# y2w-oc/CMR-Agent

Measured on AMD Instinct MI355X. Metric: registration iters/sec (KITTI 352x1216 img + 16384 pts, 1 geo forward + 10 agent steps), higher is better.
Workload: dtype f32; 1 GPU; BASELINE.json configs[1]: KittiConfig, batch 8 per GPU, 16384 pts, 352x1216 image, 10 agent steps, fp32, hash-filled weights; batch_per_gpu=8, parallelism=batch sharding, no data-path collective

## Files before the change

cmr_agent_amd/ops.py:

```python
import math
import os

import torch

from . import _lib

ACT_NONE, ACT_RELU, ACT_LRELU, ACT_GELU, ACT_ELU1 = 0, 1, 2, 3, 4
f32 = torch.float32
GRID_Y_MAX = 65535


def _stream():
    return torch.cuda.current_stream().cuda_stream


def _p(t):
    return None if t is None else t.data_ptr()


def _rows(t, name="tensor"):
    if t.dim() != 2 or t.stride(1) != 1 or t.dtype != f32 or not t.is_cuda:
        raise ValueError("%s must be a 2-D float32 device tensor with unit inner stride, got %s %s %s" % (
            name, tuple(t.shape), t.stride(), t.dtype))
    return t
# ... 3 lines not shown
    return t.stride(0) if t.shape[0] > 1 else max(t.stride(0), t.shape[1])


def _i32(t):
    if t is not None and (t.dtype != torch.int32 or not t.is_contiguous()):
        raise ValueError("row-id tensors must be contiguous int32")
    return t


LINEAR_BF16 = os.environ.get("CMR_LINEAR_BF16", "1") != "0"
LINEAR_BF16_MIN_ROWS = 16384
BN_LINEAR_BF16_FWD = os.environ.get("CMR_BN_LINEAR_BF16_FWD", "0") != "0"
BN_LINEAR_BF16_BWD = os.environ.get("CMR_BN_LINEAR_BF16_BWD", "0") != "0"


class fp32_linears:

    def __enter__(self):
        global LINEAR_BF16
        self.old, LINEAR_BF16 = LINEAR_BF16, False

    def __exit__(self, *a):
        global LINEAR_BF16
        LINEAR_BF16 = self.old


_AB_SKIP_LINEAR = os.environ.get("CMR_AB_SKIP_LINEAR", "0") == "1"
_AB_ZERO = {}
if _AB_SKIP_LINEAR:
    import sys as _sys
    print("cmr_agent_amd.ops: CMR_AB_SKIP_LINEAR=1 -- row GEMMs are NOT computed (timing experiment); every result of this process is invalid",
          file=_sys.stderr)


def linear(x1, w, bias=None, x2=None, idx2=None, div2=1, res=None, res_mod=0, act=ACT_NONE, act_param=0.0, out=None):
    _rows(x1, "x1")
    rows, k1 = x1.shape
    n_out, kw = w.shape
    k2 = 0
    if x2 is not None:
        _rows(x2, "x2")
        k2 = x2.shape[1]
    if kw != k1 + k2 or w.stride(1) != 1 or w.stride(0) < kw:
        raise ValueError("weight shape %s / strides %s do not match k1+k2=%d" % (tuple(w.shape), w.stride(), k1 + k2))
    ldw = w.stride(0) if n_out > 1 else kw
    if out is None:
        out = torch.empty((rows, n_out), dtype=f32, device=x1.device)
    _rows(out, "out")
    if res is not None:
        _rows(res, "res")
    if _AB_SKIP_LINEAR:
        key = (rows, n_out, x1.device)
        if key not in _AB_ZERO:
            _AB_ZERO[key] = torch.zeros((rows, n_out), dtype=f32, device=x1.device)
        return _AB_ZERO[key]
    if CONV_BF16 and LINEAR_BF16 and x2 is None and ldw == kw and rows >= LINEAR_BF16_MIN_ROWS and k1 in (32, 64, 128) and n_out <= 128 and n_out % 4 == 0:
        rc = _lib.call("cmr_linear_rows_bf16_f32", _p(x1), _ld(x1), k1, _p(w), kw, _p(bias), _p(res), _ld(res) if res is not None else 0,
                       int(res_mod), _p(out), _ld(out), rows, n_out, act, float(act_param), _stream(), allow_unsupported=True)
        if rc != _lib.UNSUPPORTED:
            return out
    _lib.call("cmr_linear_f32", _p(x1), _ld(x1), k1, _p(x2), _ld(x2) if x2 is not None else 0, k2, _p(_i32(idx2)),
              int(div2), _p(w), ldw, _p(bias), _p(res), _ld(res) if res is not None else 0, int(res_mod), _p(out),
              _ld(out), rows, n_out, act, float(act_param), _stream())
    return out


def cbr_block(x1, w1, b1, w2, b2, wsc, slope, x2=None, idx2=None, div2=1, rows_per_batch=None, want_y=True,
              want_colmax=False):
    _rows(x1, "x1")
    rows, k1 = x1.shape
    kx = k1 + (x2.shape[1] if x2 is not None else 0)
    ch, co = w1.shape[0], w2.shape[0]
    if w1.shape[1] != kx or w2.shape[1] != ch or (wsc is not None and tuple(wsc.shape) != (co, kx)):
        raise ValueError("cbr_block: inconsistent weight shapes")
    rpb = rows if rows_per_batch is None else rows_per_batch
    B = rows // rpb
    if want_colmax and (rpb % 32 or rows % rpb):
        return None
    y = torch.empty((rows, co), dtype=f32, device=x1.device) if want_y else None
    ntiles = (rows + 31) // 32
    part = torch.empty((ntiles, co), dtype=f32, device=x1.device) if want_colmax else None
    s1 = b1.stride(0) if b1.dim() == 2 else 0
    s2 = b2.stride(0) if b2.dim() == 2 else 0
    rc = _lib.call("cmr_cbr_block_bf16_f32" if CONV_BF16 else "cmr_cbr_block_f32", _p(x1), _ld(x1), k1, _p(x2), _ld(x2) if x2 is not None else 0, _p(_i32(idx2)),
                   int(div2), kx, ch, co, _p(w1), _p(b1), s1, _p(w2), _p(b2), s2, _p(wsc), _p(y), co, _p(part), rows, rpb,
                   float(slope), _stream(), allow_unsupported=True)
    if rc == _lib.UNSUPPORTED:
        return None
    cm = None
    if want_colmax == "partials":
        return y, part
    if want_colmax:
        cm = colmax_partials(part, B, rpb // 32)
    return y, cm


def colmax_partials(part, B, tiles_per_batch):
    co = part.shape[1]
    cm = torch.empty((B, co), dtype=f32, device=part.device)
    _lib.call("cmr_colmax_partials_f32", _p(part), _p(cm), B, int(tiles_per_batch), co, _stream())
    return cm


COLMAX_BIAS2 = os.environ.get("CMR_COLMAX_BIAS2", "fp32")


def colmax_bias2(part, B, tiles_per_batch, w1, b1, w2, b2, want_g=False):
    C = part.shape[1]
    n1, n2 = w1.shape[0], w2.shape[0]
    if COLMAX_BIAS2 == "0" or (COLMAX_BIAS2 == "fp32" and CONV_BF16) or C != 64 or n1 % 4 or n2 % 4 or not (w1.is_contiguous() and w2.is_contiguous()) or w1.shape[1] != C or w2.shape[1] != C:
        return None
    y1 = torch.empty((B, n1), dtype=f32, device=part.device)
    y2 = torch.empty((B, n2), dtype=f32, device=part.device)
    g = torch.empty((B, C), dtype=f32, device=part.device) if want_g else None
    rc = _lib.call("cmr_colmax_bias2_f32", _p(part), B, int(tiles_per_batch), C, _p(w1), _p(b1), n1, _p(w2), _p(b2), n2, _p(g), _p(y1), _p(y2), _stream(),
                   allow_unsupported=True)
    return None if rc == _lib.UNSUPPORTED else (y1, y2, g)


def layernorm64(x, gamma, beta, eps, res=None, out=None):
    _rows(x, "x")
    if out is None:
        out = torch.empty((x.shape[0], 64), dtype=f32, device=x.device)
    _lib.call("cmr_layernorm64_f32", _p(x), _ld(x), _p(gamma), _p(beta), float(eps), _p(res),
              _ld(res) if res is not None else 0, _p(out), _ld(out), x.shape[0], _stream())
    return out


CONV_BF16 = False
BF16_CHAINS = True
BF16_STORE = True
STRIDE2_FRAGS = True
WINOGRAD = True
WINO_MIN_TILES = 64


TOWER_CU_BUDGET = 160
TOWER_CU_BUDGET_F32 = 0


TOWER_SLICES_F32 = int(os.environ.get("CMR_TOWER_SLICES", "1"))


import threading

_policy = threading.local()


def _cu_budget():
    return getattr(_policy, "cu_budget", 0)


def _slices():
    return getattr(_policy, "slices", 1)


class conv_slices:

    def __init__(self, n):
        self.n = max(1, int(n))

    def __enter__(self):
        self.old, _policy.slices = _slices(), self.n

    def __exit__(self, *a):
        _policy.slices = self.old


class conv_cu_budget:

    def __init__(self, cus):
        self.cus = max(0, int(cus))

    def __enter__(self):
        self.old, _policy.cu_budget = _cu_budget(), self.cus

    def __exit__(self, *a):
        _policy.cu_budget = self.old


def conv3x3_wino(x, u, bias, cout, slope=1.0, res=None, post=None, pool=1):
    B, H, W, cin = x.shape
    if pool == 2 and (res is not None or post is not None):
        raise ValueError("conv3x3: pool=2 cannot be combined with res / post")
    if not x.is_contiguous() or tuple(u.shape) != (16, cout, cin):
        raise ValueError("conv3x3_wino: bad operand layout")
    hp, wp = (H // 2, W // 2) if pool == 2 else (H, W)
    y = torch.empty((B, hp, wp, cout), dtype=f32, device=x.device)
    _lib.call("cmr_conv3x3_wino_nhwc_f32", _p(x), B, H, W, cin, _p(u), _p(bias), _p(res), _p(post), _p(y), cout,
              float(slope), pool, _cu_budget(), _slices(), _stream())
    return y


def conv3x3_wino_stats(x, u, bias, cout):
    B, H, W, cin = x.shape
    if not (WINOGRAD and u is not None and x.dtype == f32 and x.is_contiguous() and tuple(u.shape) == (16, cout, cin)):
        return None
    parts = int(_lib.load().cmr_conv3x3_wino_stats_parts(B, H, W, cin, cout, _cu_budget(), _slices()))
    if parts <= 0:
        return None
    y = torch.empty((B, H, W, cout), dtype=f32, device=x.device)
    part = torch.empty((parts, 2, cout), dtype=f32, device=x.device)
    _lib.call("cmr_conv3x3_wino_stats_nhwc_f32", _p(x), B, H, W, cin, _p(u), _p(bias), _p(y), cout, _cu_budget(), _slices(), _p(part), parts, _stream())
    return y, part


def conv3x3_wino_bnbwd(dy, u, cout, bn_x, stat, slope):
    B, H, W, cin = dy.shape
    if not (WINOGRAD and u is not None and dy.is_contiguous() and bn_x.is_contiguous() and tuple(u.shape) == (16, cout, cin)
            and tuple(bn_x.shape) == (B, H, W, cout) and tuple(stat.shape) == (4, cout) and 0.0 <= slope <= 1.0):
        return None
# ... 1688 lines not shown
```

cmr_agent_amd/utils/workmodel.py:

```python
import torch

from .. import _lib

FP32_MFMA_PEAK = 157.3e12
HBM_PEAK = 8.0e12
RIDGE = FP32_MFMA_PEAK / HBM_PEAK
F = 4


def _linear(a):
    rows, k1, n = a["rows"], a["k1"], a["n_out"]
    k2 = a["k2"] if a["x2"] else 0
    src2 = 0
    if a["x2"]:
        src2 = rows * k2 if a["idx2"] else max(rows // max(a["div2"], 1), 1) * k2
    by = F * (rows * k1 + src2 + rows * n + n * (k1 + k2) + (rows * n if a["res"] and not a["res_mod"] else 0))
    return 2.0 * rows * (k1 + k2) * n, by


def _cbr(a):
    rows, kx, ch, co, k1 = a["rows"], a["kx"], a["ch"], a["co"], a["k1"]
    w = kx * ch + ch * co + (kx * co if a["wsc"] else 0)
    src2 = 0
    if a["x2"]:
        src2 = rows * (kx - k1) if a["idx2"] else max(rows // max(a["div2"], 1), 1) * (kx - k1)
    return 2.0 * rows * w, F * (rows * k1 + src2 + (rows * co if a["y"] else 0) + w)


def _conv(a, stride=None):
    s = a.get("stride", 1) if stride is None else stride
    B, H, W, ci, co, pool = a["B"], a["H"], a["W"], a["Cin"], a["Cout"], a.get("pool", 1)
    opix = B * ((H - 1) // s + 1) * ((W - 1) // s + 1)
    by = F * (B * H * W * ci + opix * co / (pool * pool) + (opix * co if a["res"] else 0) + 9 * ci * co)
    return 2.0 * 9 * ci * co * opix, by


def _conv_io(a):
    s = a.get("stride", 1)
    B, H, W, ci, co, pool = a["B"], a["H"], a["W"], a["Cin"], a["Cout"], a.get("pool", 1)
    opix = B * ((H - 1) // s + 1) * ((W - 1) // s + 1)
    by = ((2 if a["x_bf16"] else F) * B * H * W * ci + (2 if a["y_bf16"] else F) * opix * co / (pool * pool)
          + (2 if a.get("res_bf16") else F) * (opix * co if a["res"] else 0) + F * 9 * ci * co)
    return 2.0 * 9 * ci * co * opix, by


def _heads(a):
    w = 2 * 128 * 128 + sum(256 * a[p + "_n0"] + a[p + "_n0"] * a[p + "_n1"] + a[p + "_n1"] * a[p + "_n2"] for p in "rtv")
    return 2.0 * a["B"] * w, F * (a["B"] * a["npix"] * 128 + w)


def _vecattn(a):
    rows = a["rows"]
    if a["feat"]:
        return rows * 2.0 * (3 * 4096 + 192 + 4096 + 2 * 4096), rows * (256 + 256 + 32 + 512)
    return rows * 2.0 * (192 + 4096 + 2 * 4096), rows * (512 + 256 + 32 + 512)


WORK = {
    "cmr_linear_f32": _linear,
    "cmr_cbr_block_f32": _cbr,
    "cmr_cbr_block_bf16_f32": _cbr,
    "cmr_colmax_partials_f32": lambda a: (0, F * a["B"] * a["tiles_per_batch"] * a["C"]),
    "cmr_colmax_bias2_f32": lambda a: (2.0 * a["B"] * a["C"] * (a["n1"] + a["n2"]),
                                       F * (a["B"] * a["tiles_per_batch"] * a["C"] + (a["C"] + 1 + a["B"]) * (a["n1"] + a["n2"]))),
    "cmr_layernorm64_f32": lambda a: (0, F * a["rows"] * 64 * (3 if a["res"] else 2)),
    "cmr_conv3x3_nhwc_f32": _conv,
    "cmr_conv3x3_wino_nhwc_f32": lambda a: _conv(a, 1),
    "cmr_conv3x3_wino_stats_nhwc_f32": lambda a: (2.0 * 9 * a["Cin"] * a["Cout"] * a["B"] * a["H"] * a["W"],
                                                  F * (a["B"] * a["H"] * a["W"] * (a["Cin"] + a["Cout"]) + 9 * a["Cin"] * a["Cout"])),
    "cmr_bn_stats_from_sums_f32": lambda a: (0, F * a["parts"] * 2 * a["C"]),
    "cmr_conv3x3_wino_bnbwd_nhwc_f32": lambda a: (2.0 * 9 * a["Cin"] * a["Cout"] * a["B"] * a["H"] * a["W"],
                                                  F * (a["B"] * a["H"] * a["W"] * (a["Cin"] + 2 * a["Cout"]) + 9 * a["Cin"] * a["Cout"])),
    "cmr_bn_bwd_from_sums_f32": lambda a: (0, F * a["rows"] * a["C"] * 3),
    "cmr_conv3x3_s2_nhwc_f32": lambda a: _conv(a, 2),
    "cmr_conv3x3_bf16_nhwc_f32": _conv,
    "cmr_conv3x3_bf16io_nhwc": _conv_io,
    "cmr_conv3x3_bf16_pro_nhwc_f32": lambda a: (2.0 * 9 * a["Cin"] * a["Cout"] * a["B"] * a["H"] * a["W"],
                                                F * (a["B"] * a["H"] * a["W"] * (a["Cin"] + a["Cout"]) + 9 * a["Cin"] * a["Cout"])),
    "cmr_stem_block_f32": lambda a: (2.0 * (81 + 1728 + 192) * a["B"] * a["H"] * a["W"], a["B"] * a["H"] * a["W"] * (F * 3 + (2 if a.get("out_bf16") else F) * 64)),
    "cmr_avgpool_nhwc_f32": lambda a: (0, F * a["B"] * a["H"] * a["W"] * a["C"] * (1 + 1.0 / (a["kh"] * a["kw"]))),
    "cmr_upsample_concat_f32": lambda a: (0, F * a["B"] * a["H"] * a["W"] * (2 * a["C1"] + a["C2"] * (1 + 1.0 / a["scale"] ** 2))),
    "cmr_patchify_nhwc_f32": lambda a: (0, 2 * F * a["B"] * a["H"] * a["W"] * a["C"]),
    "cmr_transpose_f32": lambda a: (0, 2 * F * a["batch"] * a["R"] * a["Cn"]),
    "cmr_linear_rows_bf16_f32": lambda a: (2.0 * a["rows"] * a["k"] * a["n_out"], F * (a["rows"] * (a["k"] + a["n_out"] * (2 if a["res"] else 1)) + a["k"] * a["n_out"])),
    "cmr_patch_embed_f32": lambda a: (2.0 * a["B"] * (a["H"] // a["P"]) * (a["W"] // a["P"]) * a["P"] * a["P"] * a["C"] * a["n_out"],
                                     F * (a["B"] * a["H"] * a["W"] * a["C"] + a["B"] * (a["H"] // a["P"]) * (a["W"] // a["P"]) * a["n_out"] + a["P"] * a["P"] * a["C"] * a["n_out"])),
    "cmr_mha_f32": lambda a: (4.0 * a["B"] * a["Tq"] * a["Tk"] * 64, F * 64 * a["B"] * (2 * a["Tq"] + 2 * a["Tk"])),
    "cmr_mha_expf_f32": lambda a: (4.0 * a["B"] * a["Tq"] * a["Tk"] * 64, F * 64 * a["B"] * (2 * a["Tq"] + 2 * a["Tk"])),
    "cmr_mha_ln_f32": lambda a: (4.0 * a["B"] * a["Tq"] * a["Tk"] * 64 + 2.0 * 64 * a["B"] * (64 * a["Tq"] + 128 * a["Tk"]),
                                F * 64 * a["B"] * (2 * a["Tq"] + a["Tk"])),
    "cmr_la_reduce_f32": lambda a: (2.0 * a["B"] * a["S"] * 576, F * a["B"] * a["S"] * 128),
    "cmr_la_apply_f32": lambda a: (2.0 * a["B"] * a["L"] * 576, F * a["B"] * a["L"] * 128),
    "cmr_agent_heads_f32": _heads,
    "cmr_agent_heads_train_f32": _heads,
    "cmr_ln64_linear_f32": lambda a: (2.0 * 64 * (a["rows_x"] * a["n_out_x"] + (a["rows_y"] * a["n_out_y"] if a["y"] else 0)),
                                      F * (a["rows_x"] * (64 + a["n_out_x"]) + (a["rows_y"] * (64 + a["n_out_y"]) if a["y"] else 0)
                                           + 64 * (a["n_out_x"] + (a["n_out_y"] if a["y"] else 0)))),
    "cmr_ln64_linear_bf16_f32": lambda a: (2.0 * 64 * (a["rows_x"] * a["n_out_x"] + (a["rows_y"] * a["n_out_y"] if a["y"] else 0)),
                                      F * (a["rows_x"] * (64 + a["n_out_x"]) + (a["rows_y"] * (64 + a["n_out_y"]) if a["y"] else 0)
                                           + 64 * (a["n_out_x"] + (a["n_out_y"] if a["y"] else 0)))),
    "cmr_vit_out_ffn_f32": lambda a: (2.0 * a["rows"] * (4096 + 2 * 65536), F * (a["rows"] * 192 + 4096 + 2 * 65536)),
    "cmr_vit_out_ffn16_f32": lambda a: (2.0 * a["rows"] * (4096 + 2 * 65536), F * (a["rows"] * 192 + 4096 + 2 * 65536)),
    "cmr_vit_out_ffn_bf16_f32": lambda a: (2.0 * a["rows"] * (4096 + 2 * 65536), F * (a["rows"] * 192 + 4096 + 2 * 65536)),
    "cmr_la_kv_state_f32": lambda a: (2.0 * a["B"] * a["S"] * (2 * 4096 + 576), F * (a["B"] * a["S"] * 64 + 2 * 4096)),
    "cmr_la_kv_state_bf16_f32": lambda a: (2.0 * a["B"] * a["S"] * (2 * 4096 + 576), F * (a["B"] * a["S"] * 64 + 2 * 4096)),
    "cmr_la_query_layer_f32": lambda a: (2.0 * a["B"] * a["L"] * (4096 + 576 + 4096 + 16384 + 8192),
                                         F * (a["B"] * a["L"] * 128 + 2 * 4096 + 16384 + 8192)),
    "cmr_la_query_layer_bf16_f32": lambda a: (2.0 * a["B"] * a["L"] * (4096 + 576 + 4096 + 16384 + 8192),
                                         F * (a["B"] * a["L"] * 128 + 2 * 4096 + 16384 + 8192)),
    "cmr_vecattn_front_f32": _vecattn,
    "cmr_focal_metrics_f32": lambda a: (0, a["rows"] * 16),
    "cmr_circle_loss_f32": lambda a: (2.0 * a["B"] * a["n"] * a["n"] * 64, F * a["B"] * a["n"] * 128),
    "cmr_planar_to_rows_f32": lambda a: (0, F * a["B"] * a["N"] * (a["C"] + a["Cpad"])),
    "cmr_concat_rows_f32": lambda a: (0, F * a["rows"] * (2 * a["C1"] + a["C2"])),
    "cmr_index_to_global_i32": lambda a: (0, 12 * a["B"] * a["N"]),
    "cmr_csr_build_i32": lambda a: (0, 8 * a["B"] * a["n_per_batch"] + 8 * a["B"] * a["seg_per_batch"]),
    "cmr_knn16_f32": lambda a: (8.0 * a["B"] * a["M"] * a["M"], a["B"] * a["M"] * (16 + 64)),
    "cmr_nearest_f32": lambda a: (8.0 * a["B"] * a["Nq"] * a["Nc"], a["B"] * (a["Nq"] * 28 + a["Nc"] * 16)),
    "cmr_rel_pos_f32": lambda a: (0, a["rows"] * 48),
    "cmr_vecattn_prep_f32": lambda a: (0, F * a["rows"] * 64 * 6),
    "cmr_segment_softmax_f32": lambda a: (0, F * a["_rows"] * 128 + F * a["nseg"] * 64),
    "cmr_segment_reduce_f32": lambda a: (0, F * a["_rows"] * a["C"] + F * a["nseg"] * a["C"]),
    "cmr_gather_rows_f32": lambda a: (0, a["rows"] * (2 * F * a["C"] + 4)),
    "cmr_colmax_f32": lambda a: (0, F * a["B"] * a["N"] * a["C"]),
    "cmr_colmean_f32": lambda a: (0, F * a["B"] * a["N"] * a["C"]),
    "cmr_project_scatter_f32": lambda a: (0, a["B"] * a["N"] * (16 + 1 + 256 + 32)),
    "cmr_observation_finalize_f32": lambda a: (0, a["B"] * a["h"] * a["w"] * (256 + 256 + 4 + 512 + 256)),
    "cmr_pose_step_f32": lambda a: (0, a["B"] * 128),
    "cmr_to_disentangled_f32": lambda a: (0, a["B"] * 128),
    "cmr_argmax_rows_f32": lambda a: (0, a["outer"] * a["inner"] * (F * a["n"] + 8)),
    "cmr_softmax2_f32": lambda a: (0, a["rows"] * 14),
    "cmr_l2norm64_f32": lambda a: (0, a["rows"] * 512),
    "cmr_guided_match_f32": lambda a: (3.0 * 64 * (2 * a["radius"] + 1) ** 2 * a["B"] * a["N"],
                                       a["B"] * a["N"] * (12 + a["mask_bytes"] + 256 + 256 * (2 * a["radius"] + 1) ** 2 + 16)),
    "cmr_pnp_refine_f32": lambda a: ((60.0 + 112.0) * (a["iters"] + 1) * a["B"] * a["N"],
                                     (a["iters"] + 2) * a["B"] * a["N"] * (20 + a["mask_bytes"])),
    "cmr_match_subpixel_f32": lambda a: (3.0 * 64 * 5 * a["B"] * a["N"], a["B"] * a["N"] * (4 + a["mask_bytes"] + 256 + 256 * 5 + 8)),
    "cmr_match_conf_f32": lambda a: (2.0 * 2 * 64 * a["B"] * a["N"] * a["h"] * a["w"],
                                     a["B"] * (256.0 * (a["N"] + a["h"] * a["w"]) + 2.0 * a["N"] * a["h"] * a["w"])),
    "cmr_pose_score_f32": lambda a: (3.0 * 64 * (2 * a["radius"] + 1) ** 2 * a["B"] * a["N"] * a["P"],
                                     a["B"] * a["N"] * ((12 + a["mask_bytes"] + 256) * ((a["P"] + 31) // 32)
                                                        + 256.0 * (2 * a["radius"] + 1) ** 2 * a["P"])),
    "cmr_conv3x3_wgrad_f32": lambda a: (2.0 * 9 * a["Cin"] * a["Cout"] * a["B"] * a["H"] * a["W"],
                                        F * (a["B"] * a["H"] * a["W"] * (a["Cin"] + a["Cout"]) + 9 * a["Cin"] * a["Cout"])),
# ... 9 lines not shown
                                                      F * (a["B"] * a["H"] * a["W"] * (a["Cin"] + a["Cout"]) + 9 * a["Cin"] * a["Cout"])),
    "cmr_linear_bwd_rows_f32": lambda a: (4.0 * a["rows"] * a["n"] * a["k"], F * (a["rows"] * (3 * a["n"] + 3 * a["k"]) + 2 * a["n"] * a["k"])),
    "cmr_linear_wgrad_f32": lambda a: (2.0 * a["rows"] * a["n"] * a["k"], F * (a["rows"] * (a["n"] + a["k"]) + a["n"] * a["k"])),
    "cmr_adam_f32": lambda a: (0, 28 * a["n"]),
    "cmr_sgd_f32": lambda a: (0, 20 * a["n"]),
    "cmr_bn_stats_f32": lambda a: (0, F * a["rows"] * a["C"]),
    "cmr_affine_act_f32": lambda a: (0, F * a["rows"] * a["C"] * (2 + (1 if a["res"] else 0))),
    "cmr_bn_bwd_f32": lambda a: (0, F * a["rows"] * a["C"] * (3 + (1 if a["z"] else 0) + (1 if a["add"] else 0) + (1 if a["dzm"] else 0))),
    "cmr_linear_bn_fwd_f32": lambda a: (2.0 * a["rows"] * a["n"] * a["k"], F * (a["rows"] * (a["k"] + a["n"]) + a["n"] * a["k"])),
    "cmr_bn_bwd_coef_f32": lambda a: (0, F * a["rows"] * a["C"] * (2 + (1 if a["z"] else 0))),
    "cmr_bn_linear_bwd_f32": lambda a: (2.0 * a["rows"] * a["n"] * a["k"] * (2 if a["dx"] else 1),
                                        F * (a["rows"] * (a["n"] * (1 + (1 if (a["z"] and not a["mask_from_h"]) else 0) + (1 if a["stat"] else 0) + (1 if a["dzm"] else 0)) +
                                                          a["k"] * (1 + (1 if a["res"] else 0) + (1 if a["dx"] else 0))) + 2 * a["n"] * a["k"])),
    "cmr_vecattn_front_train_f32": lambda a: (2.0 * a["rows"] * (8 * 64 + 3 * 64 * 64), F * a["rows"] * (3 * 64 + 8 + 5 * 64)),
    "cmr_vecattn_front_kv_train_f32": lambda a: (2.0 * a["rows"] * (8 * 64 + 6 * 64 * 64), F * a["rows"] * (2 * 64 + 8 + 6 * 64)),
    "cmr_vecattn_mix_f32": lambda a: (0, 6 * F * a["rows"] * a["C"]),
    "cmr_vecattn_mix_bwd_f32": lambda a: (0, 4 * F * a["rows"] * a["C"]),
    "cmr_act_bwd_f32": lambda a: (0, F * a["rows"] * a["C"] * (3 + (1 if a["add"] else 0))),
    "cmr_pool_act_bwd_f32": lambda a: (0, F * a["B"] * a["H"] * a["W"] * a["C"] * (2 + 1.0 / (a["ph"] * a["pw"]))),
    "cmr_colsum_f32": lambda a: (0, F * a["B"] * a["N"] * a["C"]),
    "cmr_colmax_arg_f32": lambda a: (0, F * a["B"] * a["N"] * a["C"]),
    "cmr_add_at_arg_f32": lambda a: (0, 12 * a["B"] * a["C"]),
    "cmr_linear_bwd_small_f32": lambda a: (4.0 * a["rows"] * a["n"] * (a["k1"] + a["k2"]),
                                           F * (a["rows"] * (2 * a["n"] + 2 * (a["k1"] + a["k2"])) + 2 * a["n"] * (a["k1"] + a["k2"]))),
    "cmr_agent_loss_f32": lambda a: (0, 8 * a["B"] * (a["dr"] + a["dt"]) * a["S"]),
    "cmr_dropout_f32": lambda a: (0, 2 * F * a["rows"] * a["C"]),
    "cmr_act_f32": lambda a: (0, 2 * F * a["rows"] * a["C"]),
    "cmr_act_bwd_x_f32": lambda a: (0, 3 * F * a["rows"] * a["C"]),
    "cmr_axpy_f32": lambda a: (0, 3 * F * a["rows"] * a["C"]),
    "cmr_layernorm64_bwd_f32": lambda a: (0, 3 * F * a["rows"] * 64),
    "cmr_l2norm64_bwd_f32": lambda a: (0, 3 * F * a["rows"] * 64),
    "cmr_segment_softmax_bwd_f32": lambda a: (0, F * (a["_rows"] * 64 * 4 + a["nseg"] * 64)),
    "cmr_mha_dropout_f32": lambda a: (4.0 * a["B"] * a["Tq"] * a["Tk"] * 64, F * 64 * a["B"] * (2 * a["Tq"] + 2 * a["Tk"])),
    "cmr_mha_bwd_f32": lambda a: (10.0 * a["B"] * a["Tq"] * a["Tk"] * 64, F * 64 * a["B"] * (4 * a["Tq"] + 4 * a["Tk"])),
    "cmr_mha_dropout_bwd_f32": lambda a: (10.0 * a["B"] * a["Tq"] * a["Tk"] * 64, F * 64 * a["B"] * (4 * a["Tq"] + 4 * a["Tk"])),
    "cmr_la_bwd_f32": lambda a: (2.0 * 576 * a["B"] * (3 * a["L"] + 2 * a["S"]), F * 64 * a["B"] * (3 * a["L"] + 4 * a["S"])),
    "cmr_circle_loss_bwd_f32": lambda a: (4.0 * a["B"] * a["n"] * a["n"] * 64, 2 * F * a["B"] * a["n"] * 128),
    "cmr_focal_bwd_f32": lambda a: (0, a["rows"] * 32),
    "cmr_pack_conv3x3_f32": lambda a: (0, F * a["Cout"] * a["Cin"] * 34),
    "cmr_pack_conv3x3_slots_f32": lambda a: (0, F * a.get("_pairs", 0) * 34),
    "cmr_pack_frags_f32": lambda a: (0, 2 * F * a.get("_elems", 0)),
    "cmr_transpose_slots_f32": lambda a: (0, 2 * F * 1024 * a["total_tiles"]),
    "cmr_zero_insert2_f32": lambda a: (0, F * a["B"] * a["C"] * (a["Ho"] * a["Wo"] + a["H"] * a["W"])),
    "cmr_im2col3_f32": lambda a: (0, F * a["B"] * a["H"] * a["W"] * 40),
    "cmr_col2im3_f32": lambda a: (0, F * a["B"] * a["H"] * a["W"] * 40),
    "cmr_upsample_bwd_f32": lambda a: (0, F * a["B"] * a["H"] * a["W"] * a["C2"] * (1 + 1.0 / a["scale"] ** 2)),
    "cmr_patchify_bwd_f32": lambda a: (0, 2 * F * a["B"] * a["H"] * a["W"] * a["C"]),
    "cmr_vit_out_ffn16_train_f32": lambda a: (2.0 * a["rows"] * (4096 + 2 * 65536), F * (a["rows"] * 256 + 4096 + 2 * 65536)),
    "cmr_vit_ffn_bwd16_f32": lambda a: (2.0 * a["rows"] * (3 * 65536 + 4096), F * (a["rows"] * (7 * 64 + 2048) + 3 * 65536 + 4096)),
    "cmr_vit_lnqkv_bwd_f32": lambda a: (2.0 * 64 * (a["rows_x"] * a["k_x"] + (a["rows_y"] * a["k_y"] if a["d_y"] else 0)),
                                        F * (a["rows_x"] * (a["k_x"] + 192 + (64 if a["res"] else 0)) + (a["rows_y"] * (a["k_y"] + 192) if a["d_y"] else 0))),
    "cmr_wgrad_group_f32": lambda a: (sum(2.0 * r * n * k for r, n, k in a.get("_group", ())), F * sum(r * (n + k) + n * k for r, n, k in a.get("_group", ()))),
    "cmr_la_kv_state_train_f32": lambda a: (2.0 * a["B"] * a["S"] * (2 * 4096 + 576), F * (a["B"] * a["S"] * 192 + 2 * 4096)),
    "cmr_la_query_layer_train_f32": lambda a: (2.0 * a["B"] * a["L"] * (4096 + 576 + 4096 + 16384 + 8192), F * (a["B"] * a["L"] * (128 + 448) + 2 * 4096 + 16384 + 8192)),
    "cmr_la_mlp_bwd_f32": lambda a: (2.0 * a["rows"] * (8192 + 16384 + 4096), F * (a["rows"] * 704 + 8192 + 16384 + 4096)),
    "cmr_la_proj_bwd_f32": lambda a: (2.0 * a["_rows"] * 4096, F * a["_rows"] * 64 * 3),
    "cmr_fps_f32": lambda a: (0, a["B"] * (16 * a["N"] + 8 * a["npoint"])),
    "cmr_fps_ws_f32": lambda a: (0, a["B"] * (16 * a["N"] + 8 * a["npoint"])),
    "cmr_ball_query_f32": lambda a: (0, a["B"] * (16 * a["N"] + a["S"] * (16 + 8 * a["nsample"]))),
}

ISSUED = {"cmr_conv3x3_wino_nhwc_f32": 16.0 / 36.0, "cmr_conv3x3_wino_stats_nhwc_f32": 16.0 / 36.0, "cmr_conv3x3_wino_bnbwd_nhwc_f32": 16.0 / 36.0,
          "cmr_conv3x3_wgrad_wino_f32": 16.0 / 36.0}


def work(name, args, extra=None):
    fn = WORK.get(name)
    if fn is None:
        return None
    names = _lib.prototypes()[name][2]
    a = dict(zip(names, args))
    if extra:
        a.update(extra)
    if "_rows" not in a:
        a["_rows"] = a.get("nseg", 0) * max(a.get("fixed_len", 0), 1)
    fl, by = fn(a)
    return float(fl), float(by)


BF16_MFMA_PEAK = 2500e12


def matrix_peak(name):
    return BF16_MFMA_PEAK if "bf16" in name else FP32_MFMA_PEAK


def ideal_seconds(flops, nbytes, name=""):
    return max(flops / matrix_peak(name), nbytes / HBM_PEAK)


class CallTimer:

    def __init__(self):
        self.records = []
        self._orig = None

    def __enter__(self):
        self._orig = _lib.call

        def timed(name, *args, allow_unsupported=False, work_extra=None):
            wk = work(name, args, work_extra)
            e0, e1 = torch.cuda.Event(enable_timing=True), torch.cuda.Event(enable_timing=True)
            e0.record()
            rc = self._orig(name, *args, allow_unsupported=allow_unsupported)
            e1.record()
            if rc != _lib.UNSUPPORTED:
                self.records.append((name, e0, e1) + (wk if wk is not None else (None, None)))
            return rc
        _lib.call = timed
        return self

    def __exit__(self, *a):
        _lib.call = self._orig

    def table(self):
        agg = {}
        for name, e0, e1, fl, by in self.records:
            ms = e0.elapsed_time(e1)
            d = agg.setdefault(name, dict(name=name, calls=0, ms=0.0, flops=0.0, bytes=0.0, ideal_ms=0.0, issued_flops=0.0,
                                          ideal_issued_ms=0.0, modelled=fl is not None))
            d["calls"] += 1
            d["ms"] += ms
            if fl is not None:
                d["flops"] += fl
                d["bytes"] += by
                d["ideal_ms"] += 1e3 * ideal_seconds(fl, by, name)
                d["issued_flops"] += fl * ISSUED.get(name, 1.0)
                d["ideal_issued_ms"] += 1e3 * ideal_seconds(fl * ISSUED.get(name, 1.0), by, name)
        rows = sorted(agg.values(), key=lambda d: -d["ms"])
        for d in rows:
            d["bound"] = "mfma" if d["bytes"] and d["flops"] / d["bytes"] > matrix_peak(d["name"]) / HBM_PEAK else "hbm"
            d["frac"] = d["ideal_issued_ms"] / d["ms"] if d["ms"] > 0 else 0.0
            d["frac_algorithmic"] = d["ideal_ms"] / d["ms"] if d["ms"] > 0 else 0.0
        return rows
```

include/cmr_hip.h:

```cpp
#ifndef CMR_HIP_H
#define CMR_HIP_H
#include <stdint.h>

#ifdef __cplusplus
extern "C" {
#endif

typedef struct ihipStream_t* hipStream_t;

#define CMR_OK 0
#define CMR_EINVAL -1
#define CMR_ELAUNCH -2
#define CMR_EUNSUPPORTED -3

enum { CMR_ACT_NONE = 0, CMR_ACT_RELU = 1, CMR_ACT_LRELU = 2, CMR_ACT_GELU = 3, CMR_ACT_ELU1 = 4 };


int cmr_linear_f32(const float* x1, int64_t ld1, int k1, const float* x2, int64_t ld2, int k2, const int32_t* idx2,
                   int64_t div2, const float* w, int64_t ldw, const float* bias, const float* res, int64_t ldres,
                   int64_t res_mod, float* y, int64_t ldy, int64_t rows, int n_out, int act, float act_param,
                   hipStream_t stream);
int cmr_cbr_block_f32(const float* x1, int64_t ld1, int k1, const float* x2, int64_t ld2, const int32_t* idx2,
                      int64_t div2, int kx, int ch, int co, const float* w1, const float* b1, int64_t b1_stride,
                      const float* w2, const float* b2, int64_t b2_stride, const float* wsc, float* y, int64_t ldy,
                      float* colmax_part, int64_t rows, int64_t rows_per_batch, float slope, hipStream_t stream);
int cmr_cbr_block_bf16_f32(const float* x1, int64_t ld1, int k1, const float* x2, int64_t ld2, const int32_t* idx2,
                           int64_t div2, int kx, int ch, int co, const float* w1, const float* b1, int64_t b1_stride,
                           const float* w2, const float* b2, int64_t b2_stride, const float* wsc, float* y, int64_t ldy,
                           float* colmax_part, int64_t rows, int64_t rows_per_batch, float slope, hipStream_t stream);
int cmr_colmax_partials_f32(const float* part, float* out, int B, int tiles_per_batch, int C, hipStream_t stream);
int cmr_colmax_bias2_f32(const float* part, int B, int tiles_per_batch, int C, const float* w1, const float* b1, int n1, const float* w2,
                         const float* b2, int n2, float* g, float* y1, float* y2, hipStream_t stream);

int cmr_layernorm64_f32(const float* x, int64_t ldx, const float* gamma, const float* beta, float eps, const float* res,
                        int64_t ldres, float* y, int64_t ldy, int64_t rows, hipStream_t stream);

int cmr_conv3x3_nhwc_f32(const float* x, int B, int H, int W, int Cin, const float* w, const float* bias,
                         const float* res, const float* post, float* y, int Cout, int stride, float slope, int pool,
                         hipStream_t stream);

int cmr_conv3x3_wino_nhwc_f32(const float* x, int B, int H, int W, int Cin, const float* u, const float* bias,
                              const float* res, const float* post, float* y, int Cout, float slope, int pool,
                              int cu_budget, int slices, hipStream_t stream);
int64_t cmr_conv3x3_wino_stats_parts(int B, int H, int W, int Cin, int Cout, int cu_budget, int slices);
int cmr_conv3x3_wino_stats_nhwc_f32(const float* x, int B, int H, int W, int Cin, const float* u, const float* bias, float* y, int Cout,
                                    int cu_budget, int slices, float* part, int64_t parts, hipStream_t stream);
int cmr_conv3x3_wino_bnbwd_nhwc_f32(const float* dy, int B, int H, int W, int Cin, const float* u, float* dx, int Cout, const float* bn_x,
                                    const float* bn_stat, float bn_slope, int cu_budget, int slices, float* part, int64_t parts,
                                    hipStream_t stream);
int cmr_conv3x3_s2_nhwc_f32(const float* x, int B, int H, int W, int Cin, const float* wfrag, const float* bias, const float* res,
                            const float* post, float* y, int Cout, float slope, hipStream_t stream);
int cmr_stem_block_f32(const float* x_nchw, const float* w_a, const float* b_a, const float* w3, const float* w1,
                       const float* b_b, float* tmp_nchw, void* y_nhwc, int out_bf16, int B, int H, int W, float slope,
                       hipStream_t stream);

int cmr_avgpool_nhwc_f32(const float* x, float* y, int B, int H, int W, int C, int kh, int kw, hipStream_t stream);

int cmr_upsample_concat_f32(const float* f, const float* proxy, float* out, int B, int H, int W, int C1, int C2,
                            int scale, hipStream_t stream);

int cmr_patchify_nhwc_f32(const float* x, float* out, int B, int H, int W, int C, int P, hipStream_t stream);
int cmr_patch_embed_f32(const float* x_nhwc, int B, int H, int W, int C, int P, const float* w, int64_t ldw, const float* bias,
                        const float* res, int64_t ldres, int64_t res_mod, float* y, int64_t ldy, int n_out, hipStream_t stream);
int cmr_linear_rows_bf16_f32(const float* x, int64_t ldx, int k, const float* w, int64_t ldw, const float* bias, const float* res,
                             int64_t ldres, int64_t res_mod, float* y, int64_t ldy, int64_t rows, int n_out, int act, float act_param,
                             hipStream_t stream);

int cmr_transpose_f32(const float* x, float* y, int batch, int R, int Cn, hipStream_t stream);


int cmr_mha_f32(const float* q, int64_t ldq, const float* k, int64_t ldk, const float* v, int64_t ldv, float* o,
                int64_t ldo, int B, int Tq, int Tk, hipStream_t stream);
int cmr_mha_expf_f32(const float* q, int64_t ldq, const float* k, int64_t ldk, const float* v, int64_t ldv, float* o, int64_t ldo, int B,
                     int Tq, int Tk, hipStream_t stream);
int cmr_mha_ln_f32(const float* x, int64_t ldx, const float* y, int64_t ldy, const float* gamma, const float* beta, float eps,
                   const float* wq_frag, const float* wkv_frag, const float* bq, const float* bk, const float* bv, float* o, int64_t ldo,
                   int B, int Tq, int Tk, hipStream_t stream);
int64_t cmr_la_reduce_workspace_bytes(int B, int S);
int cmr_la_reduce_f32(const float* kf, int64_t ldk, const float* v, int64_t ldv, float* kvsum, void* workspace,
                      int64_t workspace_bytes, int B, int S, hipStream_t stream);
int cmr_la_apply_f32(const float* qf, int64_t ldq, const float* kvsum, float* msg, int64_t ldm, int B, int L, int S,
                     float eps, hipStream_t stream);

int cmr_agent_heads_f32(const float* x, int B, int npix, const float* w24, const float* b24, const float* w26,
                        const float* b26, const float* e3d,
                        const float* r_w0, const float* r_b0, const float* r_w1, const float* r_b1, const float* r_w2, const float* r_b2,
                        int r_n0, int r_n1, int r_n2, float* r_out, int r_ldo,
                        const float* t_w0, const float* t_b0, const float* t_w1, const float* t_b1, const float* t_w2, const float* t_b2,
                        int t_n0, int t_n1, int t_n2, float* t_out, int t_ldo,
                        const float* v_w0, const float* v_b0, const float* v_w1, const float* v_b1, const float* v_w2, const float* v_b2,
                        int v_n0, int v_n1, int v_n2, float* v_out, int v_ldo,
                        int num_steps, int degree_r, int degree_t, int64_t* r_act, int64_t* t_act,
                        float slope, hipStream_t stream);
int cmr_agent_heads_train_f32(const float* x, int B, int npix, const float* w24, const float* b24, const float* w26,
                              const float* b26, const float* e3d,
                              const float* r_w0, const float* r_b0, const float* r_w1, const float* r_b1, const float* r_w2, const float* r_b2,
                              int r_n0, int r_n1, int r_n2, float* r_out, int r_ldo,
                              const float* t_w0, const float* t_b0, const float* t_w1, const float* t_b1, const float* t_w2, const float* t_b2,
                              int t_n0, int t_n1, int t_n2, float* t_out, int t_ldo,
                              const float* v_w0, const float* v_b0, const float* v_w1, const float* v_b1, const float* v_w2, const float* v_b2,
                              int v_n0, int v_n1, int v_n2, float* v_out, int v_ldo,
                              float* saves, int64_t saves_floats, float slope, hipStream_t stream);
int cmr_agent_heads_t_f32(const float* x, int B, int npix, const float* w24t, const float* b24, const float* w26t, const float* b26,
                          const float* e3d,
                          const float* r_w0t, const float* r_b0, const float* r_w1t, const float* r_b1, const float* r_w2t, const float* r_b2,
                          int r_n0, int r_n1, int r_n2, float* r_out, int r_ldo,
                          const float* t_w0t, const float* t_b0, const float* t_w1t, const float* t_b1, const float* t_w2t, const float* t_b2,
                          int t_n0, int t_n1, int t_n2, float* t_out, int t_ldo,
                          const float* v_w0t, const float* v_b0, const float* v_w1t, const float* v_b1, const float* v_w2t, const float* v_b2,
                          int v_n0, int v_n1, int v_n2, float* v_out, int v_ldo,
                          int num_steps, int degree_r, int degree_t, int64_t* r_act, int64_t* t_act, float slope, hipStream_t stream);

// ... 398 lines not shown
```

Baseline: 417.7 registration iters/s.

## Add bf16x3 split-precision MFMA kernel for fp32 CBR blocks

Adds a new CBR-block kernel that splits fp32 inputs and weights into three bf16 planes and runs six bf16 MFMAs per product, emulating fp32 accuracy on the faster bf16 matrix units. Weights are pre-split into LDS once per block and input rows are prefetched one tile ahead. It is enabled by default for common shapes with kx>=64 and falls back to the existing fp32 kernel otherwise. It costs extra conversion work and LDS capacity and changes rounding slightly compared with native fp32 MFMA.

```diff
diff --git a/cmr_agent_amd/csrc/cbr_block_split.hip b/cmr_agent_amd/csrc/cbr_block_split.hip
--- /dev/null
+++ b/cmr_agent_amd/csrc/cbr_block_split.hip
@@ -0,0 +1,299 @@
+#include "cmr_common.h"
+
+namespace {
+
+typedef __bf16 cs_bf16x8 __attribute__((ext_vector_type(8)));
+
+__device__ __attribute__((aligned(16))) float cbs_zero[256] = {0.f};
+
+struct CbsArgs {
+  const float* x1; int64_t ld1;
+  const float* x2; int64_t ld2; const int32_t* idx2; int64_t div2;
+  int k1;
+  const float* w1; const float* b1; int64_t b1_stride;
+  const float* w2; const float* b2; int64_t b2_stride;
+  const float* wsc;
+  float* y; int64_t ldy;
+  float* colmax_part;
+  int64_t rows; int64_t rows_per_batch; float slope;
+};
+
+constexpr int CBS_MAXB = 16;
+constexpr int CBS_FRAG = 3 * 64;
+
+struct Cbs3 { cs_bf16x8 p0, p1, p2; };
+
+__device__ __forceinline__ float cbs_sub(float a, float b) {
+  float r;
+  asm("v_sub_f32 %0, %1, %2" : "=v"(r) : "v"(a), "v"(b));
+  return r;
+}
+
+__device__ __forceinline__ uint32_t cbs_cvt2(float lo, float hi) {
+  uint32_t r;
+  asm("v_cvt_pk_bf16_f32 %0, %1, %2" : "=v"(r) : "v"(lo), "v"(hi));
+  return r;
+}
+
+__device__ __forceinline__ Cbs3 cbs_split(const float (&v)[8]) {
+  typedef uint32_t u32x4 __attribute__((ext_vector_type(4)));
+  u32x4 p0, p1, p2;
+#pragma unroll
+  for (int j = 0; j < 4; ++j) {
+    const uint32_t a = cbs_cvt2(v[2 * j], v[2 * j + 1]);
+    const float rl = cbs_sub(v[2 * j], __builtin_bit_cast(float, a << 16)), rh = cbs_sub(v[2 * j + 1], __builtin_bit_cast(float, a & 0xffff0000u));
+    const uint32_t b = cbs_cvt2(rl, rh);
+    const float sl = cbs_sub(rl, __builtin_bit_cast(float, b << 16)), sh = cbs_sub(rh, __builtin_bit_cast(float, b & 0xffff0000u));
+    p0[j] = a;
+    p1[j] = b;
+    p2[j] = cbs_cvt2(sl, sh);
+  }
+  return {__builtin_bit_cast(cs_bf16x8, p0), __builtin_bit_cast(cs_bf16x8, p1), __builtin_bit_cast(cs_bf16x8, p2)};
+}
+
+__device__ __forceinline__ void cbs_put(cs_bf16x8* frag_lane, const float (&v)[8]) {
+  const Cbs3 s = cbs_split(v);
+  frag_lane[0] = s.p0;
+  frag_lane[64] = s.p1;
+  frag_lane[128] = s.p2;
+}
+
+__device__ __forceinline__ f32x16 cbs_mma6(const cs_bf16x8* frag_lane, const Cbs3& x, f32x16 acc) {
+  const cs_bf16x8 w0 = frag_lane[0], w1 = frag_lane[64], w2 = frag_lane[128];
+  acc = __builtin_amdgcn_mfma_f32_32x32x16_bf16(w2, x.p0, acc, 0, 0, 0);
+  acc = __builtin_amdgcn_mfma_f32_32x32x16_bf16(w0, x.p2, acc, 0, 0, 0);
+  acc = __builtin_amdgcn_mfma_f32_32x32x16_bf16(w1, x.p1, acc, 0, 0, 0);
+  acc = __builtin_amdgcn_mfma_f32_32x32x16_bf16(w1, x.p0, acc, 0, 0, 0);
+  acc = __builtin_amdgcn_mfma_f32_32x32x16_bf16(w0, x.p1, acc, 0, 0, 0);
+  acc = __builtin_amdgcn_mfma_f32_32x32x16_bf16(w0, x.p0, acc, 0, 0, 0);
+  return acc;
+}
+
+template <int KX, int CH, int CO, bool CONV_SC>
+__global__ __launch_bounds__(512) void cbr_block_split_kernel(const CbsArgs a) {
+  constexpr int S1 = (KX + 15) / 16;
+  constexpr int T1 = (CH + 31) / 32, T2 = CO / 32;
+  constexpr int CHP = 32 * T1;
+  constexpr int S2 = 2 * T1;
+  extern __shared__ __attribute__((aligned(16))) unsigned char smem_raw[];
+  cs_bf16x8* W1f = reinterpret_cast<cs_bf16x8*>(smem_raw);
+  cs_bf16x8* W2f = W1f + T1 * S1 * CBS_FRAG;
+  cs_bf16x8* Wsf = W2f + T2 * S2 * CBS_FRAG;
+  float* B1s = reinterpret_cast<float*>(Wsf + (CONV_SC ? T2 * S1 * CBS_FRAG : 0));
+  float* B2s = B1s + CBS_MAXB * CHP;
+  const int tid = threadIdx.x, lane = tid & 63;
+  const int wave = __builtin_amdgcn_readfirstlane(tid >> 6);
+  const int h = lane >> 5, l31 = lane & 31;
+  const uint32_t rows = (uint32_t)a.rows, rpb = (uint32_t)a.rows_per_batch;
+  const int nb1 = a.b1_stride > 0 ? (int)((rows + rpb - 1) / rpb) : 1, nb2 = a.b2_stride > 0 ? (int)((rows + rpb - 1) / rpb) : 1;
+  for (int e = tid; e < T1 * S1 * 64; e += 512) {
+    const int ln = e & 63, s = (e >> 6) % S1, t = (e >> 6) / S1;
+    const int n = 32 * t + (ln & 31), k0 = 16 * s + 8 * (ln >> 5);
+    float v[8];
+#pragma unroll
+    for (int j = 0; j < 8; ++j) v[j] = (n < CH && k0 + j < KX) ? a.w1[(int64_t)n * KX + k0 + j] : 0.f;
+    cbs_put(W1f + (e >> 6) * CBS_FRAG + ln, v);
+  }
+  for (int e = tid; e < T2 * S2 * 64; e += 512) {
+    const int ln = e & 63, s = (e >> 6) % S2, n = (e >> 6) / S2;
+    const int t = s >> 1, s2 = s & 1, hh = ln >> 5;
+    const int co = 32 * n + (ln & 31);
+    float v[8];
+#pragma unroll
+    for (int j = 0; j < 8; ++j) {
+      const int c = 32 * t + (j & 3) + 8 * (2 * s2 + (j >> 2)) + 4 * hh;
+      v[j] = c < CH ? a.w2[(int64_t)co * CH + c] : 0.f;
+    }
+    cbs_put(W2f + (e >> 6) * CBS_FRAG + ln, v);
+  }
+  if (CONV_SC)
+    for (int e = tid; e < T2 * S1 * 64; e += 512) {
+      const int ln = e & 63, s = (e >> 6) % S1, n = (e >> 6) / S1;
+      const int co = 32 * n + (ln & 31), k0 = 16 * s + 8 * (ln >> 5);
+      float v[8];
+#pragma unroll
+      for (int j = 0; j < 8; ++j) v[j] = k0 + j < KX ? a.wsc[(int64_t)co * KX + k0 + j] : 0.f;
+      cbs_put(Wsf + (e >> 6) * CBS_FRAG + ln, v);
+    }
+  for (int e = tid; e < nb1 * CHP; e += 512) B1s[e] = (e % CHP) < CH ? a.b1[(int64_t)(e / CHP) * a.b1_stride + e % CHP] : 0.f;
+  for (int e = tid; e < nb2 * CO; e += 512) B2s[e] = a.b2[(int64_t)(e / CO) * a.b2_stride + e % CO];
+  __syncthreads();
+
+  const uint32_t ntiles = (rows + 31) / 32, tstride = gridDim.x * 8;
+  const float* x2b = a.x2 ? a.x2 : a.x1;
+  const int32_t* izero = reinterpret_cast<const int32_t*>(cbs_zero);
+  auto load_idx = [&](uint32_t tile) -> int32_t {
+    const uint32_t row = tile * 32 + l31;
+    const uint32_t ok = (a.idx2 != nullptr && tile < ntiles && row < rows) ? 1u : 0u;
+    return (a.idx2 ? a.idx2 : izero)[ok * row];
+  };
+  struct RowPtr { const float* p1; const float* p2; };
+  auto row_ptr = [&](uint32_t tile, int32_t idxv) -> RowPtr {
+    uint32_t row = tile * 32 + l31;
+    row = (tile < ntiles && row < rows) ? row : 0;
+    const int64_t r2 = a.idx2 ? (int64_t)idxv : (int64_t)(row / (uint32_t)a.div2);
+    return {a.x1 + (int64_t)row * a.ld1, x2b + r2 * a.ld2 - a.k1};
+  };
+  auto load_x = [&](const RowPtr& r, f32x4 (&lo)[S1], f32x4 (&hi)[S1]) {
+#pragma unroll
+    for (int s = 0; s < S1; ++s) {
+      constexpr bool FULL = KX % 16 == 0;
+      const int c0 = 16 * s + 8 * h, c1 = c0 + 4;
+      lo[s] = *reinterpret_cast<const f32x4*>((FULL || c0 < KX) ? (c0 < a.k1 ? r.p1 : r.p2) + c0 : cbs_zero);
+      hi[s] = *reinterpret_cast<const f32x4*>((FULL || c1 < KX) ? (c1 < a.k1 ? r.p1 : r.p2) + c1 : cbs_zero);
+    }
+  };
+
+  uint32_t tile = blockIdx.x * 8 + wave;
+  f32x4 xlo[S1], xhi[S1], nlo[S1], nhi[S1];
+  int32_t idn = load_idx(tile);
+  RowPtr rc = row_ptr(tile, idn);
+  load_x(rc, xlo, xhi);
+  idn = load_idx(tile + tstride);
+  for (; tile < ntiles; tile += tstride) {
+    const uint32_t row = tile * 32 + l31;
+    const bool valid = row < rows;
+    const uint32_t batch = (valid ? row : 0) / rpb;
+    const RowPtr rn = row_ptr(tile + tstride, idn);
+    load_x(rn, nlo, nhi);
+    idn = load_idx(tile + 2 * tstride);
+    Cbs3 xb[S1];
+#pragma unroll
+    for (int s = 0; s < S1; ++s) {
+      const float v[8] = {xlo[s][0], xlo[s][1], xlo[s][2], xlo[s][3], xhi[s][0], xhi[s][1], xhi[s][2], xhi[s][3]};
+      xb[s] = cbs_split(v);
+    }
+    f32x16 hid[T1];
+#pragma unroll
+    for (int t = 0; t < T1; ++t)
+#pragma unroll
+      for (int r = 0; r < 16; ++r) hid[t][r] = 0.f;
+#pragma unroll
+    for (int s = 0; s < S1; ++s)
+#pragma unroll
+      for (int t = 0; t < T1; ++t) hid[t] = cbs_mma6(W1f + (t * S1 + s) * CBS_FRAG + lane, xb[s], hid[t]);
+    {
+      const float* b1 = B1s + (a.b1_stride > 0 ? batch : 0) * CHP + 4 * h;
+#pragma unroll
+      for (int t = 0; t < T1; ++t)
+#pragma unroll
+        for (int q = 0; q < 4; ++q) {
+          const f32x4 bv = *reinterpret_cast<const f32x4*>(b1 + 32 * t + 8 * q);
+#pragma unroll
+          for (int e = 0; e < 4; ++e) {
+            const float v = hid[t][4 * q + e] + bv[e];
+            hid[t][4 * q + e] = v > 0.f ? v : v * a.slope;
+          }
+        }
+    }
+    f32x16 acc[T2];
+#pragma unroll
+    for (int n = 0; n < T2; ++n)
+#pragma unroll
+      for (int r = 0; r < 16; ++r) acc[n][r] = 0.f;
+    if (CONV_SC) {
+#pragma unroll
+      for (int s = 0; s < S1; ++s)
+#pragma unroll
+        for (int n = 0; n < T2; ++n) acc[n] = cbs_mma6(Wsf + (n * S1 + s) * CBS_FRAG + lane, xb[s], acc[n]);
+    }
+#pragma unroll
+    for (int t = 0; t < T1; ++t)
+#pragma unroll
+      for (int s2 = 0; s2 < 2; ++s2) {
+        float v[8];
+#pragma unroll
+        for (int j = 0; j < 8; ++j) v[j] = hid[t][8 * s2 + j];
+        const Cbs3 hb = cbs_split(v);
+#pragma unroll
+        for (int n = 0; n < T2; ++n) acc[n] = cbs_mma6(W2f + (n * S2 + 2 * t + s2) * CBS_FRAG + lane, hb, acc[n]);
+      }
+    const float* b2 = B2s + (a.b2_stride > 0 ? batch : 0) * CO + 4 * h;
+    f32x4 ov[T2][4];
+#pragma unroll
+    for (int n = 0; n < T2; ++n)
+#pragma unroll
+      for (int q = 0; q < 4; ++q) {
+        const f32x4 bv = *reinterpret_cast<const f32x4*>(b2 + n * 32 + q * 8);
+        f32x4 sc = {0.f, 0.f, 0.f, 0.f};
+        if (!CONV_SC && 32 * n + 8 * q < KX) {
+          const int c = 32 * n + 8 * q + 4 * h;
+          sc = *reinterpret_cast<const f32x4*>((c < a.k1 ? rc.p1 : rc.p2) + c);
+        }
+#pragma unroll
+        for (int e = 0; e < 4; ++e) {
+          float s = acc[n][4 * q + e] + bv[e];
+          if (!CONV_SC) s += sc[e];
+          ov[n][q][e] = s > 0.f ? s : s * a.slope;
+        }
+      }
+#pragma unroll
+    for (int n = 0; n < T2; ++n)
+#pragma unroll
+      for (int q = 0; q < 4; ++q) cmr_pin(ov[n][q]);
+    if (a.y && valid) {
+      float* yrow = a.y + (int64_t)row * a.ldy + 4 * h;
+#pragma unroll
+      for (int n = 0; n < T2; ++n)
+#pragma unroll
+        for (int q = 0; q < 4; ++q) *reinterpret_cast<f32x4*>(yrow + n * 32 + q * 8) = ov[n][q];
+    }
+    if (a.colmax_part) {
+      const bool whole = tile * 32 + 32 <= rows;
+#pragma unroll
+      for (int n = 0; n < T2; ++n)
+#pragma unroll
+        for (int q = 0; q < 4; ++q) {
+          f32x4 v = ov[n][q];
+#pragma unroll
+          for (int e = 0; e < 4; ++e) v[e] = cmr_rowmax32(whole || valid ? v[e] : -INFINITY);
+          if (l31 == 16) *reinterpret_cast<f32x4*>(a.colmax_part + (int64_t)tile * CO + n * 32 + q * 8 + 4 * h) = v;
+        }
+    }
+    rc = rn;
+#pragma unroll
+    for (int s = 0; s < S1; ++s) {
+      xlo[s] = nlo[s];
+      xhi[s] = nhi[s];
+    }
+  }
+}
+
+template <int KX, int CH, int CO, bool CONV_SC>
+int launch_cbs(const CbsArgs& a, hipStream_t stream) {
+  constexpr int S1 = (KX + 15) / 16, T1 = (CH + 31) / 32, T2 = CO / 32, S2 = 2 * T1;
+  constexpr size_t smem = (size_t)(T1 * S1 + T2 * S2 + (CONV_SC ? T2 * S1 : 0)) * CBS_FRAG * sizeof(cs_bf16x8) +
+                          (size_t)CBS_MAXB * (32 * T1 + CO) * sizeof(float);
+  static_assert(smem <= 160 * 1024, "three weight planes must fit in LDS");
+  static CmrSmemCache granted{};
+  if (cmr_grant_smem(reinterpret_cast<const void*>(cbr_block_split_kernel<KX, CH, CO, CONV_SC>), smem, granted) != CMR_OK) return CMR_ELAUNCH;
+  const int64_t ntiles = (a.rows + 31) / 32;
+  int64_t grid = (ntiles + 7) / 8;
+  if (grid > 256) grid = 256;
+  hipLaunchKernelGGL((cbr_block_split_kernel<KX, CH, CO, CONV_SC>), dim3((unsigned)grid), dim3(512), smem, stream, a);
+  return cmr_launch_status();
+}
+
+}
+
+extern "C" int cmr_cbr_block_split_f32(const float* x1, int64_t ld1, int k1, const float* x2, int64_t ld2, const int32_t* idx2,
+                                       int64_t div2, int kx, int ch, int co, const float* w1, const float* b1, int64_t b1_stride,
+                                       const float* w2, const float* b2, int64_t b2_stride, const float* wsc, float* y, int64_t ldy,
+                                       float* colmax_part, int64_t rows, int64_t rows_per_batch, float slope, hipStream_t stream) {
+  CMR_REQUIRE(x1 && w1 && b1 && w2 && b2 && (y || colmax_part) && rows > 0 && rows_per_batch > 0);
+  CMR_REQUIRE(k1 > 0 && k1 % 4 == 0 && k1 <= kx && (k1 == kx || x2) && ld1 % 4 == 0 && cmr_aligned16(x1));
+  if (x2) CMR_REQUIRE(ld2 % 4 == 0 && cmr_aligned16(x2) && (idx2 || div2 >= 1));
+  if (y) CMR_REQUIRE(ldy % 4 == 0 && cmr_aligned16(y));
+  CMR_REQUIRE(cmr_aligned16(w1) && cmr_aligned16(w2) && cmr_aligned16(b1) && cmr_aligned16(b2) && b1_stride % 4 == 0 &&
+              b2_stride % 4 == 0 && (!wsc || cmr_aligned16(wsc)) && (!colmax_part || cmr_aligned16(colmax_part)));
+  const CbsArgs a{x1, ld1, x2, ld2, idx2, div2 < 1 ? 1 : div2, k1, w1, b1, b1_stride, w2, b2, b2_stride, wsc, y, ldy,
+                  colmax_part, rows, rows_per_batch, slope};
+  const bool conv = wsc != nullptr;
+  if (rows >= (int64_t)0x7fffffc0 || ((b1_stride > 0 || b2_stride > 0) && (rows + rows_per_batch - 1) / rows_per_batch > CBS_MAXB))
+    return CMR_EUNSUPPORTED;
+  if (kx == 64 && ch == 64 && co == 64 && !conv) return launch_cbs<64, 64, 64, false>(a, stream);
+  if (kx == 64 && ch == 128 && co == 64 && conv) return launch_cbs<64, 128, 64, true>(a, stream);
+  if (kx == 64 && ch == 128 && co == 128 && !conv) return launch_cbs<64, 128, 128, false>(a, stream);
+  if (kx == 8 && ch == 8 && co == 64 && conv) return launch_cbs<8, 8, 64, true>(a, stream);
+  return CMR_EUNSUPPORTED;
+}
diff --git a/cmr_agent_amd/ops.py b/cmr_agent_amd/ops.py
--- a/cmr_agent_amd/ops.py
+++ b/cmr_agent_amd/ops.py
@@ -109,9 +109,13 @@
     part = torch.empty((ntiles, co), dtype=f32, device=x1.device) if want_colmax else None
     s1 = b1.stride(0) if b1.dim() == 2 else 0
     s2 = b2.stride(0) if b2.dim() == 2 else 0
-    rc = _lib.call("cmr_cbr_block_bf16_f32" if CONV_BF16 else "cmr_cbr_block_f32", _p(x1), _ld(x1), k1, _p(x2), _ld(x2) if x2 is not None else 0, _p(_i32(idx2)),
-                   int(div2), kx, ch, co, _p(w1), _p(b1), s1, _p(w2), _p(b2), s2, _p(wsc), _p(y), co, _p(part), rows, rpb,
-                   float(slope), _stream(), allow_unsupported=True)
+    args = (_p(x1), _ld(x1), k1, _p(x2), _ld(x2) if x2 is not None else 0, _p(_i32(idx2)), int(div2), kx, ch, co, _p(w1), _p(b1), s1, _p(w2),
+            _p(b2), s2, _p(wsc), _p(y), co, _p(part), rows, rpb, float(slope), _stream())
+    rc = _lib.UNSUPPORTED
+    if CBR_SPLIT and not CONV_BF16 and kx >= 64:
+        rc = _lib.call("cmr_cbr_block_split_f32", *args, allow_unsupported=True)
+    if rc == _lib.UNSUPPORTED:
+        rc = _lib.call("cmr_cbr_block_bf16_f32" if CONV_BF16 else "cmr_cbr_block_f32", *args, allow_unsupported=True)
     if rc == _lib.UNSUPPORTED:
         return None
     cm = None
@@ -154,6 +158,7 @@
     return out
 
 
+CBR_SPLIT = os.environ.get("CMR_CBR_SPLIT", "1") != "0"
 CONV_BF16 = False
 BF16_CHAINS = True
 BF16_STORE = True
diff --git a/cmr_agent_amd/utils/workmodel.py b/cmr_agent_amd/utils/workmodel.py
--- a/cmr_agent_amd/utils/workmodel.py
+++ b/cmr_agent_amd/utils/workmodel.py
@@ -60,6 +60,7 @@
     "cmr_linear_f32": _linear,
     "cmr_cbr_block_f32": _cbr,
     "cmr_cbr_block_bf16_f32": _cbr,
+    "cmr_cbr_block_split_f32": _cbr,
     "cmr_colmax_partials_f32": lambda a: (0, F * a["B"] * a["tiles_per_batch"] * a["C"]),
     "cmr_colmax_bias2_f32": lambda a: (2.0 * a["B"] * a["C"] * (a["n1"] + a["n2"]),
                                        F * (a["B"] * a["tiles_per_batch"] * a["C"] + (a["C"] + 1 + a["B"]) * (a["n1"] + a["n2"]))),
@@ -235,6 +236,8 @@
 
 
 def matrix_peak(name):
+    if "_split_" in name:
+        return BF16_MFMA_PEAK / 6
     return BF16_MFMA_PEAK if "bf16" in name else FP32_MFMA_PEAK
 
 
diff --git a/include/cmr_hip.h b/include/cmr_hip.h
--- a/include/cmr_hip.h
+++ b/include/cmr_hip.h
@@ -28,6 +28,10 @@
                            int64_t div2, int kx, int ch, int co, const float* w1, const float* b1, int64_t b1_stride,
                            const float* w2, const float* b2, int64_t b2_stride, const float* wsc, float* y, int64_t ldy,
                            float* colmax_part, int64_t rows, int64_t rows_per_batch, float slope, hipStream_t stream);
+int cmr_cbr_block_split_f32(const float* x1, int64_t ld1, int k1, const float* x2, int64_t ld2, const int32_t* idx2,
+                            int64_t div2, int kx, int ch, int co, const float* w1, const float* b1, int64_t b1_stride,
+                            const float* w2, const float* b2, int64_t b2_stride, const float* wsc, float* y, int64_t ldy,
+                            float* colmax_part, int64_t rows, int64_t rows_per_batch, float slope, hipStream_t stream);
 int cmr_colmax_partials_f32(const float* part, float* out, int B, int tiles_per_batch, int C, hipStream_t stream);
 int cmr_colmax_bias2_f32(const float* part, int B, int tiles_per_batch, int C, const float* w1, const float* b1, int n1, const float* w2,
                          const float* b2, int n2, float* g, float* y1, float* y2, hipStream_t stream);
```

Measured after the change: 432.8 registration iters/s (median of 6 runs). 1.04x the previous value.
